# dzhang314/DZOptimization.jl

Measured on AMD Instinct MI355X. Metric: step!() calls/sec and achieved HBM GB/s, L-BFGS n=10^7 m=20 fp64, higher is better.
Workload: dtype f64

## Files before the change

### dzoptimization.jl_amd/__init__.py

```python
from __future__ import annotations

import ctypes as C
import os
import subprocess
import sys

import numpy as np

_HERE = os.path.dirname(os.path.abspath(__file__))
LIB_PATH = os.environ.get("DZO_LIB_PATH") or os.path.join(_HERE, "libdzo_hip.so")
INCLUDE_DIR = os.path.join(os.path.dirname(_HERE), "include")

F32, F64 = 0, 1
ROSENBROCK2D, ROSENBROCK_CHAIN, QUADRATIC, LSE, QUADRATIC_CHAIN = 0, 1, 2, 3, 4
PAIRWISE_LJ = 5
RADIAL_LENNARD_JONES = 0
RADIAL_MORSE_RHO6, RADIAL_MORSE_RHO14 = 2, 3
TWOLOOP_CHAIN, TWOLOOP_GRAM = 0, 1
LINE_SEARCH_BACKTRACKING, LINE_SEARCH_WOLFE = 0, 1
STEP_NULL, STEP_GRADIENT_DESCENT, STEP_BFGS = 0, 1, 2

_ERR = {1: "invalid argument", 2: "HIP runtime error", 3: "reference @assert", 4: "out of memory",
        5: "unsupported", 6: "bad call sequence", 7: "more candidates than the capacity"}

# ... 1915 lines not shown
    rho_history = property(lambda s: s._hist(lib().dzo_lbfgs_get_rho))
    alpha_history = property(lambda s: s._hist(lib().dzo_lbfgs_get_alpha))

    def set_two_loop_mode(self, mode):
        _check(lib().dzo_lbfgs_set_two_loop_mode(self.h, mode))

    def set_max_halvings(self, v):
        _check(lib().dzo_lbfgs_set_max_halvings(self.h, v))

    def set_safeguards(self, descent_check=False, steepest_descent_fallback=False):
        _check(lib().dzo_lbfgs_set_safeguards(self.h, int(descent_check), int(steepest_descent_fallback)))

    def set_line_search(self, kind, c1=0.0, c2=0.0, max_evals=0):
        _check(lib().dzo_lbfgs_set_line_search(self.h, int(kind), c1, c2, int(max_evals)))

    last_step_length = property(lambda s: s._s(2))
    history_resets = property(lambda s: s._i(8))
    descent_resets = property(lambda s: s._i(9))
    last_step_kind = property(lambda s: s._i(10))
    single_pass_steps = property(lambda s: s._i(11))
    single_pass_rejections = property(lambda s: s._i(12))
    single_pass_retries = property(lambda s: s._i(13))
    ring_layout = property(lambda s: s._i(14))
    tile_arrangement = property(lambda s: s._i(15))
    pass_recomputes_gradients = property(lambda s: bool(s._i(16)))
    pass_register_sets = property(lambda s: s._i(17))
    host_write_checks = property(lambda s: s._i(18))

    def compute_step_direction(self, sync=True):
        _check(lib().dzo_lbfgs_direction(self.h))
        return self.step_direction if sync else None

    def set_history(self, S, Y, rho=None, iteration_count=None):
        S, Y = _as_dev(S, self.dtype), _as_dev(Y, self.dtype)
        k = S.shape[0] if len(S.shape) == 2 else 0
        rp = None if rho is None else (C.c_double * k)(*[float(r) for r in rho])
        _check(lib().dzo_lbfgs_set_history(self.h, k, S.ptr, Y.ptr, rp, k if iteration_count is None else iteration_count))

    def begin_search(self):
        _check(lib().dzo_lbfgs_begin_search(self.h))

    def trial(self, t):
# ... 432 lines not shown
```

### dzoptimization.jl_amd/csrc/dzo_lbfgs.hip

```cpp
#include <cmath>
#include <cstdlib>
#include <limits>
#include <map>
#include <mutex>
#include <type_traits>
#include <utility>

#include "dzo_lbfgs_plan.h"
#include "dzo_optcore.h"
#include "dzo_rosen.h"

namespace dzo {

static_assert(kPlanWaves == kWaves && kPlanMaxHistory == kMaxHistory && kPlanMaxPartialBlocks == kMaxPartialBlocks,
              "dzo_lbfgs_plan.h restates these constants of dzo_common.h");

struct SlotMap {
    uint8_t slot[kMaxHistory];
};

}

struct dzo_lbfgs_s {
    dzo::OptCore core;
// ... 30 lines not shown
    int32_t wolfe_max_evals = 40;
    double last_step_length = 0;
    int64_t history_resets = 0, descent_resets = 0;
    int32_t last_step_kind = 0;
    bool reset_on_push = false;
    void *xt = nullptr, *gt = nullptr;
    bool single_pass = true;
    bool gram_ready = false;
    int gram_ready_grid = 0;
    bool scalars_ready = false;
    void *twin_slab = nullptr, *x_twin = nullptr, *g_twin = nullptr, *d_alloc = nullptr;
    void *x_user = nullptr, *g_user = nullptr;
    bool unsettled = false;
    std::recursive_mutex mu;
    int64_t single_pass_steps = 0, single_pass_rejections = 0, single_pass_retries = 0;
    bool fused_post = true;

    int device = 0;
    int32_t nslots = 0;
    int slot_of(int i) const { return ((newest - i) % nslots + nslots) % nslots; }
    int spare() const { return (newest + 1) % nslots; }
    int64_t pair_stride = 0;
    bool blocked = false;
    int64_t rowbytes = 0, ring_rows = 0;
    int64_t tile_stride = dzo::kTileBytes;
    size_t ring_bytes = 0;
    void *dx_lin = nullptr, *dg_lin = nullptr;
    bool lin_stale = false;
    void *export_slab = nullptr;
    bool points = false;
// ... 688 lines not shown
template <typename T> __device__ __forceinline__ T decor_grad(const PointDecor<T> &d, T g, T x) {
    const T g2 = dfma(d.two_lambda, x, g);
    g = d.l2_on ? g2 : g;
    const bool pushed_back = (x <= d.bg_lo && g >= (T)0) || (x >= d.bg_hi && g <= (T)0);
    return pushed_back ? (T)0 : g;
}
template <typename T> __device__ __forceinline__ T decor_clamp(const PointDecor<T> &d, T v) {
    return v < d.cons_lo ? d.cons_lo : (v > d.cons_hi ? d.cons_hi : v);
}

template <typename T> struct FusedParams {
    int64_t n;
    int k;
    int k_next;
    T t;
    T t_half;
    const T *x, *g;
    T *x_out, *g_out;
    T *d;
    const double *alpha, *coef, *scale;
    T *ring;
    uint32_t rowbytes;
    uint32_t soff[kFusedMaxK + 1];
    uint32_t new_off;
    uint32_t ystride;
    double *gram_partials;
    double *obj_partials;
    int32_t *changed;
    int nt_tiles;
    int stage_rows;
    int store_d;
    int prio;
    int leftover_even;
    int debug_skip;
    PointDecor<T> dec;
    T obj_lambda;
};

template <typename T> static inline bool fused_params_ok(const FusedParams<T> &fp, bool pair) {
    const bool common = fp.ring && fp.alpha && fp.coef && fp.scale && fp.gram_partials && fp.obj_partials && fp.changed && fp.rowbytes != 0 && fp.n > 0;
    return common && (!pair || (fp.x && fp.g && fp.x_out && fp.g_out && fp.d)) && (pair || fp.d);
}

// ... 82 lines not shown
#pragma unroll
        for (int i = K - 1; i >= 0; --i) {
            const T c = c_s[i];
#pragma unroll
            for (int j = 0; j < N; ++j) q[j] = dfma(c, sv[i][j], q[j]);
        }
        T xn[N];
#pragma unroll
        for (int j = 0; j < N; ++j) {
            xn[j] = dfma(p.t, q[j], xo[j]);
            diff |= owner && !is_equal(xn[j], xo[j]);
        }
        {
            T xh[N];
#pragma unroll
            for (int j = 0; j < N; ++j) xh[j] = dfma(p.t_half, q[j], xo[j]);
            const T xhnext = lane_next<T>(xh[0]);
#pragma unroll
            for (int j = 0; j < N; ++j) {
                const T xq = j + 1 < N ? xh[(j + 1) % N] : xhnext;
                if (owner && e0 + j + 1 < p.n) fobj_h += rosen_term<T>(xh[j], xq);
            }
        }
        const T xprev = lane_prev<T>(xn[N - 1]);
        const T xnext = lane_next<T>(xn[0]);
        T gn[N], sn[N], yn[N];
#pragma unroll
        for (int j = 0; j < N; ++j) {
            const T xp = j > 0 ? xn[(j + N - 1) % N] : xprev;
            const T xq = j + 1 < N ? xn[(j + 1) % N] : xnext;
            gn[j] = rosen_grad_elem<T>(e0 + j, p.n, xp, xn[j], xq);
// ... 130 lines not shown
    __shared__ int64_t stage_row_s[kWaves][40];
    extern __shared__ __attribute__((aligned(16))) char stage_lds[];
    const int lane = threadIdx.x & 63;
    const int wave = threadIdx.x >> 6;
    const int stage_rows = p.stage_rows;
    constexpr bool kWriteG = !(DZO_PP_REGRAD != 0 && !FIRST);
    constexpr int kStageTiles = kWriteG ? 2 : 1;
    char *stage = stage_lds + (size_t)wave * stage_rows * (kStageTiles * kTileBytes);
    int staged = 0;
    const int k = p.k, kn = p.k_next;
    if (threadIdx.x < K) {
        a_s[threadIdx.x] = threadIdx.x < k ? (T)(-p.alpha[threadIdx.x]) : (T)0;
        c_s[threadIdx.x] = threadIdx.x < k ? (T)(-p.coef[threadIdx.x]) : (T)0;
    }
    constexpr bool kRegrad = DZO_PP_REGRAD != 0 && !FIRST;
    __syncthreads();
    const bool scaled = k > 0;
    const T scale = scaled ? (T)p.scale[0] : (T)1;
    const int64_t nvec = (p.n + N - 1) / N;
    const int64_t rows = (nvec + kOwn - 1) / kOwn;
    const int64_t row_end = rows;
    const int64_t stride = (int64_t)gridDim.x * kWaves;
    const int pstride = (int)gridDim.x;
    const int pcol = (int)blockIdx.x;
    TreeSum<kGramValues * (K + 1)> dots;
    dots.init();
    double fobj = 0, fobj_h = 0;
    double fsq = 0, fsq_h = 0;
    bool diff = false;
    auto byte_offset = [&](int64_t row) -> uint32_t {
// ... 97 lines not shown
            }
            if (scaled) {
#pragma unroll
                for (int j = 0; j < N; ++j) q[j] = scale * q[j];
            }
#pragma unroll
            for (int i = K - 1; i >= 0; --i) {
                const T c = c_s[i];
#pragma unroll
                for (int j = 0; j < N; ++j) q[j] = dfma(c, xv[i][j] - xv[i + 1][j], q[j]);
            }
        }
        T xn[N];
#pragma unroll
        for (int j = 0; j < N; ++j) {
            xn[j] = dfma(p.t, q[j], xv[0][j]);
            diff |= owner && !is_equal(xn[j], xv[0][j]);
            if constexpr (DEC) { const T cl = decor_clamp<T>(p.dec, xn[j]); xn[j] = e0 + j < p.n ? cl : xn[j]; }
        }
        {
            T xh[N];
#pragma unroll
            for (int j = 0; j < N; ++j) {
                xh[j] = dfma(p.t_half, q[j], xv[0][j]);
                if constexpr (DEC) {
                    const T cl = decor_clamp<T>(p.dec, xh[j]); xh[j] = e0 + j < p.n ? cl : xh[j];
                    if (owner) fsq_h = __builtin_fma((double)xh[j], (double)xh[j], fsq_h);
                }
            }
            const T xhnext = lane_next0<T>(xh[0]);
#pragma unroll
            for (int j = 0; j < N; ++j) {
                const T xq = j + 1 < N ? xh[(j + 1) % N] : xhnext;
                if (owner && Obj::has_term(e0 + j, p.n)) fobj_h += Obj::term(rc[j], xh[j], xq);
            }
        }
        const T xprev = lane_prev0<T>(xn[N - 1]);
        const T xnext = lane_next0<T>(xn[0]);
        T gn[N], sn[N], yn[N];
// ... 142 lines not shown
        const double *wflat = &wacc[0][0][0];
        constexpr int ws = kGramValues * (kFusedMaxK + 1);
        const double r = (wflat[v] + wflat[ws + v]) + (wflat[2 * ws + v] + wflat[3 * ws + v]);
        p.gram_partials[(int64_t)v * pstride + pcol] = r;
    }
    block_raise_flag(diff, p.changed, &lds_flag);
    const double fo = block_sum(fobj, lds);
    const double fh = block_sum(fobj_h, lds);
    if (threadIdx.x == 0) { p.obj_partials[pcol] = fo; p.obj_partials[pstride + pcol] = fh; }
    if constexpr (DEC) {
        const double so = block_sum(fsq, lds);
        const double sh = block_sum(fsq_h, lds);
        if (threadIdx.x == 0) { p.obj_partials[2 * pstride + pcol] = so; p.obj_partials[3 * pstride + pcol] = sh; }
    }
    if ((p.debug_skip & 1024) && blockIdx.x < 1024) { if (lane == 0) g_dev_wave_times[(blockIdx.x * kWaves + wave) * 2 + 1] = wall_clock64(); }
}

constexpr int kLseMaxK = 24;
template <typename T> struct LseParams {
    int64_t n;
    int k, k_next;
    T t;
    T *ring;
    uint32_t rowbytes;
    uint32_t soff[kLseMaxK + 1];
    uint32_t new_off, c_off;
    uint8_t slot[kLseMaxK + 1];
    uint8_t new_slot;
    double *pscal;
    double lambda;
// ... 1273 lines not shown
    DeviceScope scope(o->device);
    DZO_TRY(lbfgs_settle(o));
    DZO_HIP(hipStreamSynchronize(o->core.stream));
    return DZO_OK;
}


template <typename P> static int32_t pass_trial_launch(OptCore &c, void (*kern)(P), int grid, size_t dyn_lds, const P &p, int attempt) {
    if (!c.flag_armed) DZO_HIP(hipMemsetAsync(c.flag(), 0, sizeof(int32_t), c.stream));
    c.flag_armed = false;
    DZO_TIMED(attempt == 0 ? "lbfgs_single_pass" : "lbfgs_single_pass_retry", c.stream);
    hipLaunchKernelGGL(kern, dim3(grid), dim3(kBlock), dyn_lds, c.stream, p);
    return DZO_OK;
}

static int32_t gram_reduce_decide_launch(dzo_lbfgs_s *o, int k_next, const double *obj_partials, int grid, const double *l2_partials) {
    OptCore &c = o->core;
    {
        DZO_TIMED("lbfgs_gram_reduce", c.stream);
        const int nvals = kGramValues * k_next;
        DecideArgs da = decide_args(c, obj_partials, grid, 1.0);
        da.partials2 = obj_partials + grid;
        if (l2_partials) { da.l2_partials = l2_partials; da.l2_partials2 = l2_partials + grid; da.l2_lambda = o->ring_dec.l2; }
        hipLaunchKernelGGL(gram_reduce_decide_kernel, dim3(nvals + 1), dim3(kBlock), 0, c.stream, (const double *)o->gram_partials, grid, gram_vals(o),
                           nvals, da);
        c.flag_armed = true;
    }
    DZO_HIP(hipGetLastError());
    return DZO_OK;
}

static int32_t next_scalars_gated(dzo_lbfgs_s *o, int k_next) {
    const int sv_newest = o->newest, sv_k = o->k;
    o->newest = o->spare(); o->k = k_next;
    const int32_t rc = gram_finish_launch(o, 0, true, gram_vals(o), true, o->core.status());
    o->newest = sv_newest; o->k = sv_k;
    return rc;
}
// ... 16 lines not shown
    if (v.k > 0) { o->d_stale = true; o->dview_k = v.k; o->dview_newest = v.newest; }
}

template <typename T> static void fused_fill_params(dzo_lbfgs_s *o, FusedParams<T> &fp, int k, int view_newest) {
    OptCore &c = o->core;
    memset(&fp, 0, sizeof(fp));
    fp.n = c.n; fp.k = k; fp.k_next = k < o->m ? k + 1 : o->m;
    fp.d = (T *)o->d;
    fp.ring = (T *)o->S; fp.rowbytes = (uint32_t)o->rowbytes;
    fp.new_off = ring_tile_off(o, o->spare()); fp.ystride = (uint32_t)o->tile_stride;
    fp.alpha = o->alpha; fp.coef = o->coef; fp.scale = o->scale;
    for (int j = 0; j <= kFusedMaxK; ++j) fp.soff[j] = ring_tile_off(o, ring_view_slot(o, view_newest, j < k ? j : k));
    fp.gram_partials = o->gram_partials;
    fp.obj_partials = c.problem->scratch;
    fp.changed = c.flag();
    fp.dec = point_decor<T>(o->ring_dec);
    fp.obj_lambda = (T)o->ring_obj_lambda;
}

template <typename T> static int32_t points_end_stuck(dzo_lbfgs_s *o, RingView view) {
    o->core.is_stuck = true;
    direction_pending(o, view);
    if (o->k > 0) {
        DZO_TRY(lbfgs_ensure_g(o, o->slot_of(0))); DZO_TRY(lbfgs_ensure_g(o, o->slot_of(1)));
        ring_gather_diff<T>(o, o->y_slot_v(o->slot_of(0)), o->y_slot_v(o->slot_of(1)), o->dg_lin);
    }
    ring_gather<T>(o, o->s_slot_v(o->newest), o->dx_lin);
    DZO_HIP(hipGetLastError());
    o->lin_stale = false;
    return DZO_OK;
// ... 30 lines not shown
    fp.obj_partials = c.problem->scratch;
    fp.changed = c.flag();
    fp.debug_skip = tune_int("DZO_TUNE_SP_DEBUG", 0);
    const int pass_k = pair_pass_k(o->m);
    void (*kern)(FusedParams<T>) = pass_k == 8 ? lbfgs_single_pass_kernel<T, 8>
                                   : pass_k == 16 ? lbfgs_single_pass_kernel<T, 16>
                                   : lbfgs_single_pass_kernel<T, 20>;
    if constexpr (std::is_same<T, double>::value) {
        if ((fp.debug_skip & 256) && o->m > 16) kern = lbfgs_single_pass_kernel<double, 20, true>;
    }
    const int grid = pass_grid(rows, (int64_t)ctx().cus * resident_blocks((const void *)kern), o->gram_grid, kPairPassGridCap);
    DZO_REQUIRE(fused_params_ok<T>(fp, true), DZO_ERR_STATE, "single-pass step: a null operand (ring %p, x %p, g %p, twins %p %p, d %p)",
                (void *)fp.ring, (const void *)fp.x, (const void *)fp.g, (void *)fp.x_out, (void *)fp.g_out, (void *)fp.d);
    double t = 1.0;
    for (int attempt = 0;; ++attempt) {
    fp.t = (T)t; fp.t_half = (T)round_to_dtype(c.dtype, t * 0.5);
    DZO_TRY(pass_trial_launch(c, kern, grid, 0, fp, attempt));
    DZO_TRY(gram_reduce_decide_launch(o, fp.k_next, fp.obj_partials, grid, nullptr));
    DZO_TRY(next_scalars_gated(o, fp.k_next));
    DZO_TRY(core_wait_decision(c));
    const int32_t status = c.host_status();
    if (attempt == 0) { c.last_trials = 0; o->single_pass_steps += 1; }
    if (status == 2) {
        c.is_stuck = true;
        if (o->lin_stale && o->k > 0) { ring_gather<T>(o, o->y_slot_v(o->newest), o->dg_lin); o->lin_stale = false; }
        DZO_HIP(hipMemcpyAsync(c.dx, c.x, (size_t)c.n * sizeof(T), hipMemcpyDeviceToDevice, c.stream));
        DZO_HIP(hipGetLastError());
        return DZO_OK;
    }
    c.last_trials += 1;
    if (status == 1) {
// ... 31 lines not shown
        DZO_PP(24, false, 2, true, 0) DZO_PP(16, false, 2, true, 0) DZO_PP(20, false, 2, true, 0) DZO_PP(12, false, 2, true, 0)
        DZO_PP(18, false, 1, false, 0) DZO_PP(20, false, 1, false, 0) DZO_PP(16, false, 1, false, 0) DZO_PP(14, false, 1, false, 0) DZO_PP(12, false, 1, false, 0) DZO_PP(10, false, 1, false, 0) DZO_PP(8, false, 1, false, 0) DZO_PP(6, false, 1, false, 0)
        DZO_PP(22, false, 2, false, 0) DZO_PP(24, false, 2, false, 0) DZO_PP(16, false, 2, false, 0) DZO_PP(20, false, 2, false, 0) DZO_PP(12, false, 2, false, 0) DZO_PP(8, false, 2, false, 0)
    } else {
        DZO_PP(8, true, 2, true, 0) DZO_PP(8, true, 2, false, 0) DZO_PP(8, true, 2, false, 1)
        DZO_PP(8, false, 1, false, 1) DZO_PP(12, false, 1, false, 1)
        DZO_PP(16, false, 2, false, 1) DZO_PP(20, false, 2, false, 1) DZO_PP(12, false, 2, false, 1)
        DZO_PP(8, false, 1, true, 0) DZO_PP(12, false, 1, true, 0)
        DZO_PP(16, false, 2, true, 0) DZO_PP(20, false, 2, true, 0) DZO_PP(12, false, 2, true, 0)
        DZO_PP(10, false, 1, false, 0) DZO_PP(12, false, 1, false, 0) DZO_PP(8, false, 1, false, 0) DZO_PP(6, false, 1, false, 0)
        DZO_PP(16, false, 2, false, 0) DZO_PP(20, false, 2, false, 0) DZO_PP(12, false, 2, false, 0) DZO_PP(8, false, 2, false, 0)
    }
#undef DZO_PP
    return nullptr;
}
template <typename T> static void (*point_pass_kernel_for(dzo_lbfgs_s *o, bool first))(FusedParams<T>) {
    return point_pass_kernel_of<T>(point_pass_variant(o->m, o->core.dtype, point_one_set(o->m, o->core.dtype, o->point_sets),
                                                      o->ring_dec.any(), o->ring_obj, first));
}

template <typename T> static int32_t lbfgs_materialize_d_t(dzo_lbfgs_s *o) {
    OptCore &c = o->core;
    hipStream_t s = c.stream;
    FusedParams<T> fp;
    fused_fill_params<T>(o, fp, o->dview_k, o->dview_newest);
    fp.k_next = 1; fp.t = (T)1; fp.t_half = (T)0.5;
    fp.store_d = 1;
    fp.debug_skip = 1 | 64;
    fp.stage_rows = 1;
    void (*kern)(FusedParams<T>) = point_pass_kernel_for<T>(o, false);
    DZO_REQUIRE(kern, DZO_ERR_STATE, "direction on demand: no point-pass kernel for history_length %d", o->m);
    const int grid = points_grid<T>(o, kern);
    DZO_REQUIRE(fused_params_ok<T>(fp, false), DZO_ERR_STATE, "direction on demand: a null operand (ring %p, d %p)", (void *)fp.ring, (void *)fp.d);
    {
        DZO_TIMED("lbfgs_direction_on_demand", s);
        hipLaunchKernelGGL(kern, dim3(grid), dim3(kBlock), 0, s, fp);
    }
    DZO_HIP(hipMemsetAsync(c.flag(), 0, sizeof(int32_t), s));
    c.flag_armed = true;
    DZO_HIP(hipGetLastError());
    o->d_stale = false;
// ... 35 lines not shown
        o->stage_kern = (const void *)kern; o->stage_bytes = stage_bytes;
    }
    if (o->stage_small && fp.stage_rows > point_stage_small_rows(pl.stage_tiles)) {
        fp.stage_rows = point_stage_small_rows(pl.stage_tiles);
        stage_bytes = point_stage_bytes(fp.stage_rows, pl.stage_tiles);
    }
    const int grid = points_grid<T>(o, kern, stage_bytes);
    const int pgrid = grid;
    DZO_REQUIRE(fused_params_ok<T>(fp, false), DZO_ERR_STATE, "point pass: a null operand (ring %p, d %p, scalars %p %p %p)",
                (void *)fp.ring, (void *)fp.d, (const void *)fp.alpha, (const void *)fp.coef, (const void *)fp.scale);
    o->d_stale = false;
    const RingView view{k, o->newest};
    const double *l2_partials = o->ring_dec.l2 != 0.0 ? fp.obj_partials + 2 * pgrid : nullptr;
    c.last_trials = 0;
    o->single_pass_steps += 1;
    int64_t halvings = 0;
    double t = 1.0;
    for (int attempt = 0;; ++attempt) {
        fp.t = (T)t; fp.t_half = (T)round_to_dtype(c.dtype, t * 0.5);
        DZO_TRY(pass_trial_launch(c, kern, grid, stage_bytes, fp, attempt));
        DZO_TRY(gram_reduce_decide_launch(o, fp.k_next, fp.obj_partials, pgrid, l2_partials));
        DZO_TRY(next_scalars_gated(o, fp.k_next));
        DZO_TRY(core_wait_decision(c));
        const int32_t status = c.host_status();
        if (status == 2) return points_end_stuck<T>(o, view);
        c.last_trials += 1;
        if (status == 1) {
            return points_accept(o, view, round_to_dtype(c.dtype, c.host[0]), (k == 0) || DZO_PP_REGRAD == 0);
        }
        if (attempt == 0) o->single_pass_rejections += 1;
        auto halve = [&]() -> bool {
            t = round_to_dtype(c.dtype, t * 0.5);
            return !(c.max_halvings > 0 && ++halvings >= c.max_halvings);
        };
        bool go_on = halve();
        const double f_half = round_to_dtype(c.dtype, c.host[1]);
        if (go_on && !(f_half < c.f)) {
            c.last_trials += 1;
            go_on = halve();
        }
        if (!go_on) return points_end_stuck<T>(o, view);
        o->single_pass_retries += 1;
    }
}

template <typename T> static void lse_fill_params(dzo_lbfgs_s *o, LseParams<T> &lp, int k, int view_newest) {
    OptCore &c = o->core;
    memset(&lp, 0, sizeof(lp));
    lp.n = c.n; lp.k = k; lp.k_next = k < o->m ? k + 1 : o->m;
// ... 292 lines not shown
int32_t dzo_lbfgs_destroy(dzo_lbfgs_t o) {
    if (!o) return DZO_OK;
    DeviceScope scope(o->device);
    if (o->core.stream && o->x_user) (void)lbfgs_settle(o);
    unsettled_retire(o);
    if (o->core.stream) (void)hipStreamSynchronize(o->core.stream);
    if (o->S) (void)hipFree(o->S);
    if (o->d_alloc) (void)hipFree(o->d_alloc);
    if (o->twin_slab) (void)hipFree(o->twin_slab);
    if (o->dx_lin) (void)hipFree(o->dx_lin);
    if (o->dg_lin) (void)hipFree(o->dg_lin);
    if (o->export_slab) (void)hipFree(o->export_slab);
    if (o->xt) (void)hipFree(o->xt);
    if (o->gt) (void)hipFree(o->gt);
    if (o->gram_ticket) (void)hipFree(o->gram_ticket);
    core_free(o->core);
    delete o;
    return DZO_OK;
}

int32_t dzo_lbfgs_create_callbacks(dzo_constraint_fn constraint, dzo_objective_fn objective, dzo_gradient_fn gradient,
                                   void *cb_ctx, int64_t n, int32_t history_length, int32_t dtype, void *x_dev,
                                   double initial_step_length, dzo_lbfgs_t *out) {
    DZO_TRY(require_init());
    DZO_REQUIRE(objective && gradient && x_dev && out, DZO_ERR_INVALID, "null argument");
    DZO_REQUIRE(dtype == DZO_F32 || dtype == DZO_F64, DZO_ERR_INVALID, "bad dtype %d", dtype);
    DZO_TRY(require_same_backend("LBFGSOptimizer", "src/DZOptimization.jl:410,420", x_dev, "initial_point", nullptr, ""));
    if (constraint) DZO_REQUIRE(constraint(cb_ctx, x_dev) != 0, DZO_ERR_ASSERT,
                                "@assert constraint_function!(initial_point) (src/DZOptimization.jl:412-414)");
    const double f0 = objective(cb_ctx, x_dev);
// ... 148 lines not shown
    switch (what) {
    case 0: *value = o->core.is_stuck ? 1 : 0; break;
    case 1: *value = o->core.iteration_count; break;
    case 2: *value = o->core.n; break;
    case 3: *value = o->m; break;
    case 4: *value = o->k; break;
    case 5: *value = o->core.last_trials; break;
    case 6: *value = o->mode; break;
    case 7: *value = o->core.dtype; break;
    case 8: *value = o->history_resets; break;
    case 9: *value = o->descent_resets; break;
    case 10: *value = o->last_step_kind; break;
    case 11: *value = o->single_pass_steps; break;
    case 12: *value = o->single_pass_rejections; break;
    case 13: *value = o->single_pass_retries; break;
    case 14: *value = o->points ? 2 : (o->blocked ? 1 : 0); break;
    case 15: *value = o->blocked ? (o->tile_stride == kTileBytes ? 1 : 2) : 0; break;
    case 16: *value = (o->points && DZO_PP_REGRAD != 0) ? 1 : 0; break;
    case 18: *value = o->host_write_checks; break;
    case 17: { int sets = 0; if (o->points) { sets = point_one_set(o->m, o->core.dtype, o->point_sets) ? 1 : 2; } *value = sets; break; }
    default: set_error("dzo_lbfgs_get_i: unknown field %d", what); return DZO_ERR_INVALID;
    }
    return DZO_OK;
}

int32_t dzo_lbfgs_get_s(dzo_lbfgs_t o, int32_t what, double *value) {
    DZO_REQUIRE(o && value, DZO_ERR_INVALID, "null argument");
    DZO_REQUIRE(what >= 0 && what <= 2, DZO_ERR_INVALID, "unknown field %d", what);
    *value = what == 0 ? o->core.f : what == 1 ? o->core.df : o->last_step_length;
    return DZO_OK;
// ... 11 lines not shown
    DZO_REQUIRE(o, DZO_ERR_INVALID, "null optimizer");
    DZO_REQUIRE(kind == DZO_LINE_SEARCH_BACKTRACKING || kind == DZO_LINE_SEARCH_WOLFE, DZO_ERR_INVALID,
                "unknown line search %d", kind);
    DZO_REQUIRE(!(c1 > 0 && c2 > 0) || c1 < c2, DZO_ERR_INVALID, "Wolfe constants need 0 < c1 < c2 < 1");
    DZO_REQUIRE(c2 < 1.0, DZO_ERR_INVALID, "Wolfe constants need 0 < c1 < c2 < 1");
    DeviceScope scope(o->device);
    o->line_search = kind;
    if (c1 > 0) o->wolfe_c1 = round_to_dtype(o->core.dtype, c1);
    if (c2 > 0) o->wolfe_c2 = round_to_dtype(o->core.dtype, c2);
    if (max_evals > 0) o->wolfe_max_evals = max_evals;
    return DZO_OK;
}

int32_t dzo_lbfgs_set_s(dzo_lbfgs_t o, int32_t what, double value) {
    DZO_REQUIRE(o, DZO_ERR_INVALID, "null optimizer");
    DZO_REQUIRE(what >= 0 && what <= 2, DZO_ERR_INVALID, "unknown field %d", what);
    (what == 0 ? o->core.f : what == 1 ? o->core.df : o->last_step_length) = round_to_dtype(o->core.dtype, value);
    return DZO_OK;
}

int32_t dzo_lbfgs_set_stuck(dzo_lbfgs_t o, int32_t is_stuck) {
    DZO_REQUIRE(o, DZO_ERR_INVALID, "null optimizer");
    o->core.is_stuck = is_stuck != 0;
    return DZO_OK;
}

static int32_t lbfgs_field_ptr(dzo_lbfgs_t o, int32_t what, int32_t idx, bool hand_out, void **ptr_dev) {
    DZO_TRY(lbfgs_settle(o, hand_out));
    if (what == 1 || what == 3) DZO_TRY(lbfgs_refresh_lin(o));
    if (what == 4) DZO_TRY(lbfgs_materialize_d(o));
    if ((what == 5 || what == 6) && o->blocked) {
// ... 221 lines not shown
```

### dzoptimization.jl_amd/csrc/dzo_lbfgs_plan.h

```cpp
#pragma once

#include <cstddef>
#include <cstdint>

#include "../../include/dzo.h"

namespace dzo {

constexpr int kPlanWaves = 4, kPlanMaxHistory = 64, kPlanMaxPartialBlocks = 2048;

constexpr int kGramValues = 5;
constexpr int kRowOwn = 62;
constexpr int kRowLead = (64 - kRowOwn) / 2;
constexpr int kTileBytes = 64 * 16;
constexpr int kPairMaxK = 20;
static inline int point_max_k(int32_t dtype) { return dtype == DZO_F64 ? 24 : 20; }
constexpr int kFusedMaxK = 24;
constexpr int kStreamU = 4;

static inline int64_t plan_dtype_size(int32_t dtype) { return dtype == DZO_F64 ? 8 : 4; }

struct RingDecor {
    double l2 = 0; bool bg_on = false; double bg_lo = 0, bg_hi = 0; bool cons_on = false; double cons_lo = 0, cons_hi = 0;
    bool any() const { return l2 != 0.0 || bg_on || cons_on; }
// ... 203 lines not shown
static inline int point_stage_small_rows(int stage_tiles) { return 14 / stage_tiles; }
static inline PointLaunch point_pass_launch(int64_t n, int32_t dtype, int m, int k, int point_sets, bool regrad,
                                            int stage_rows_knob, int prio_knob, int64_t plain_mb) {
    PointLaunch p;
    p.nt_tiles = 2 * n * plan_dtype_size(dtype) > (plain_mb << 20) ? 1 : 0;
    p.one_set = point_one_set(m, dtype, point_sets) && k > 0;
    p.prio = p.one_set ? (prio_knob != 0 ? 1 : 0) : 0;
    p.stage_tiles = (k == 0 || !regrad) ? 2 : 1;
    p.stage_max = (p.one_set ? 72 : 144) / (4 * p.stage_tiles);
    p.stage_rows = stage_rows_knob < 1 ? 1 : stage_rows_knob;
    if (p.stage_rows > p.stage_max) p.stage_rows = p.stage_max;
    p.stage_bytes = point_stage_bytes(p.stage_rows, p.stage_tiles);
    return p;
}

}
```

### dzoptimization.jl_amd/csrc/dzo_optcore.h

```cpp
#pragma once
#include "dzo_common.h"
#include "dzo_problems.h"

namespace dzo {

struct OptCore {
    int64_t n = 0;
    int32_t dtype = DZO_F64;
    hipStream_t stream = nullptr;

    dzo_constraint_fn constraint = nullptr;
    dzo_objective_fn objective = nullptr;
    dzo_gradient_fn gradient = nullptr;
    void *cb_ctx = nullptr;
    dzo_problem_s *problem = nullptr;
    bool box_on = false; double box_lo = 0, box_hi = 0;

    bool is_stuck = false;
    int64_t iteration_count = 0;
    void *x = nullptr;
    void *dx = nullptr;
    double f = 0;
    double df = 0;
    void *g = nullptr;
// ... 5 lines not shown
    double *host_dev = nullptr;
    bool flag_armed = false;
    double ticket = 0;
    int64_t max_halvings = 4096;
    int64_t last_trials = 0;
    bool search_open = false;
    bool defer_delta = false;
    int32_t (*speculative_tail)(void *self, const int32_t *gate) = nullptr;
    void *speculative_self = nullptr;
    hipEvent_t decided = nullptr;

    double *partials() const { return ws; }
    double *result() const { return ws + 2 * kMaxPartialBlocks; }
    int32_t *flag() const { return reinterpret_cast<int32_t *>(ws + 2 * kMaxPartialBlocks + 4); }
    int32_t *status() const { return reinterpret_cast<int32_t *>(ws + 2 * kMaxPartialBlocks + 3); }
    int32_t host_status() const { return reinterpret_cast<const int32_t *>(host + 3)[0]; }
    bool has_objective() const { return objective != nullptr || problem != nullptr; }
    bool has_gradient() const { return gradient != nullptr || problem != nullptr; }
};

int32_t core_alloc(OptCore &c);
void core_free(OptCore &c);

inline double round_to_dtype(int32_t dtype, double v) { return dtype == DZO_F32 ? (double)(float)v : v; }

int32_t core_begin_search(OptCore &c);
int32_t core_trial(OptCore &c, double t, const void *dir, bool fuse_objective, int32_t *changed,
                   double *f_new, bool *f_valid);
int32_t core_accept(OptCore &c, double f_new);
int32_t core_reject(OptCore &c);
// ... 6 lines not shown

struct DecideArgs {
    double *result;
    const double *partials;
    const double *partials2;
    int64_t count;
    double scale;
    int32_t *changed;
    double f_cur;
    int to_f32;
    int32_t *status;
    double *host_out;
    double ticket;
    const double *l2_partials = nullptr, *l2_partials2 = nullptr;
    double l2_lambda = 0;
};
DecideArgs decide_args(OptCore &c, const double *partials, int64_t count, double scale);

__device__ __forceinline__ void decide_body(const DecideArgs &a, double *lds) {
    double f_new;
    double f_second = 0;
    const int32_t ch_early = threadIdx.x == 0 ? *a.changed : 0;
    if (a.partials && a.partials2) {
        __shared__ double lds2[2 * kWaves];
        double v[2] = {0, 0}, out[2];
        for (int64_t i = threadIdx.x; i < a.count; i += kBlock) { v[0] += a.partials[i]; v[1] += a.partials2[i]; }
        block_sum_multi<2>(v, lds2, out);
        f_new = a.scale * out[0];
        f_second = a.scale * out[1];
        if (a.l2_partials) {
            double w[2] = {0, 0}, ss[2];
            for (int64_t i = threadIdx.x; i < a.count; i += kBlock) { w[0] += a.l2_partials[i]; w[1] += a.l2_partials2[i]; }
            block_sum_multi<2>(w, lds2, ss);
            if (a.to_f32) {
                f_new = (double)((float)f_new + (float)a.l2_lambda * (float)ss[0]);
                f_second = (double)((float)f_second + (float)a.l2_lambda * (float)ss[1]);
            } else {
// ... 8 lines not shown
            for (int64_t i = threadIdx.x; i < a.count; i += kBlock) v += a.partials[i];
            f_new = a.scale * block_sum(v, lds);
            if (threadIdx.x == 0) a.result[0] = f_new;
        } else {
            f_new = a.result[0];
        }
        if (a.partials2) {
            double v = 0;
            for (int64_t i = threadIdx.x; i < a.count; i += kBlock) v += a.partials2[i];
            f_second = a.scale * block_sum(v, lds);
        }
    }
    if (threadIdx.x == 0) {
        const double f_raw = f_new;
        if (a.to_f32) f_new = (double)(float)f_new;
        const int32_t ch = ch_early;
        int32_t st = 0;
        if (ch == 0) st = 2;
        else if (f_new < a.f_cur) st = 1;
        *a.status = st;
        *a.changed = 0;
        const unsigned long long sw = (unsigned long long)(uint32_t)st, cw = (unsigned long long)(uint32_t)ch;
        unsigned long long *ho = reinterpret_cast<unsigned long long *>(a.host_out);
        auto put = [&](int i, unsigned long long w) { __hip_atomic_store(ho + i, w, __ATOMIC_RELAXED, __HIP_MEMORY_SCOPE_SYSTEM); };
        put(0, seal_bits(f_raw));
        put(1, seal_bits(f_second));
        put(2, 0ull); put(5, 0ull);
        put(3, sw);
        put(4, cw);
        put(6, seal_bits(f_raw) ^ seal_bits(f_second) ^ sw ^ cw ^ seal_bits(a.ticket));
        put(7, seal_bits(a.ticket));
    }
}

}
```

Measured before the change: 2736.

## Add sampled point probe to predict full-step rejection and swap trial order

Adds a small sampling kernel that estimates the objective change at the full step over a strided subset of rows before the fused single-pass trial. If the probe predicts rejection, the pass evaluates the half step as the primary candidate and the full step as the secondary one. The decide logic is extended to handle swapped passes, including a false-alarm status that triggers a retry. A credit scheme arms the probe only for a while after a first-trial rejection. The aim is to avoid wasted full passes over the large history ring when the unit step keeps being rejected, at the cost of an extra small kernel launch and more complex control flow.

```diff
diff --git a/dzoptimization.jl_amd/__init__.py b/dzoptimization.jl_amd/__init__.py
--- a/dzoptimization.jl_amd/__init__.py
+++ b/dzoptimization.jl_amd/__init__.py
@@ -1953,6 +1953,9 @@
     def set_line_search(self, kind, c1=0.0, c2=0.0, max_evals=0):
         _check(lib().dzo_lbfgs_set_line_search(self.h, int(kind), c1, c2, int(max_evals)))
 
+    def set_point_probe(self, mode):
+        _check(lib().dzo_lbfgs_set_s(self.h, 3, float(mode)))
+
     last_step_length = property(lambda s: s._s(2))
     history_resets = property(lambda s: s._i(8))
     descent_resets = property(lambda s: s._i(9))
@@ -1965,6 +1968,10 @@
     pass_recomputes_gradients = property(lambda s: bool(s._i(16)))
     pass_register_sets = property(lambda s: s._i(17))
     host_write_checks = property(lambda s: s._i(18))
+    probe_runs = property(lambda s: s._i(19))
+    probe_hits = property(lambda s: s._i(20))
+    point_probe = property(lambda s: s._i(22))
+    probe_false_alarms = property(lambda s: s._i(21))
 
     def compute_step_direction(self, sync=True):
         _check(lib().dzo_lbfgs_direction(self.h))
diff --git a/dzoptimization.jl_amd/csrc/dzo_lbfgs.hip b/dzoptimization.jl_amd/csrc/dzo_lbfgs.hip
--- a/dzoptimization.jl_amd/csrc/dzo_lbfgs.hip
+++ b/dzoptimization.jl_amd/csrc/dzo_lbfgs.hip
@@ -68,6 +68,10 @@
     bool unsettled = false;
     std::recursive_mutex mu;
     int64_t single_pass_steps = 0, single_pass_rejections = 0, single_pass_retries = 0;
+    int probe_mode = dzo::kProbeRule;
+    int probe_credit = 0;
+    double *probe_ws = nullptr;
+    int64_t probe_runs = 0, probe_hits = 0, probe_false_alarms = 0;
     bool fused_post = true;
 
     int device = 0;
@@ -786,7 +790,7 @@
     int k;
     int k_next;
     T t;
-    T t_half;
+    T t_other;
     const T *x, *g;
     T *x_out, *g_out;
     T *d;
@@ -799,6 +803,10 @@
     double *gram_partials;
     double *obj_partials;
     int32_t *changed;
+    int probe_use;
+    int probe_blocks;
+    double *probe_partials;
+    int32_t *pass_mode;
     int nt_tiles;
     int stage_rows;
     int store_d;
@@ -911,7 +919,7 @@
         {
             T xh[N];
 #pragma unroll
-            for (int j = 0; j < N; ++j) xh[j] = dfma(p.t_half, q[j], xo[j]);
+            for (int j = 0; j < N; ++j) xh[j] = dfma(p.t_other, q[j], xo[j]);
             const T xhnext = lane_next<T>(xh[0]);
 #pragma unroll
             for (int j = 0; j < N; ++j) {
@@ -1072,6 +1080,19 @@
         c_s[threadIdx.x] = threadIdx.x < k ? (T)(-p.coef[threadIdx.x]) : (T)0;
     }
     constexpr bool kRegrad = DZO_PP_REGRAD != 0 && !FIRST;
+    T t_p = p.t, t_o = p.t_other;
+    if constexpr (!FIRST) {
+        int swapped = p.probe_use == kProbeUseSwap ? 1 : 0;
+        if (p.probe_use == kProbeUseRule) {
+            double ps = 0, pa = 0;
+            for (int i = lane; i < p.probe_blocks; i += 64) { ps += p.probe_partials[i]; pa += p.probe_partials[p.probe_blocks + i]; }
+            ps = wave_sum_all(ps); pa = wave_sum_all(pa);
+            swapped = probe_predicts_reject(ps, pa) ? 1 : 0;
+        }
+        swapped = __builtin_amdgcn_readfirstlane(swapped);
+        if (swapped) { t_p = p.t_other; t_o = p.t; }
+        if (swapped && blockIdx.x == 0 && threadIdx.x == 0) *p.pass_mode = 1;
+    }
     __syncthreads();
     const bool scaled = k > 0;
     const T scale = scaled ? (T)p.scale[0] : (T)1;
@@ -1199,7 +1220,7 @@
         T xn[N];
 #pragma unroll
         for (int j = 0; j < N; ++j) {
-            xn[j] = dfma(p.t, q[j], xv[0][j]);
+            xn[j] = dfma(t_p, q[j], xv[0][j]);
             diff |= owner && !is_equal(xn[j], xv[0][j]);
             if constexpr (DEC) { const T cl = decor_clamp<T>(p.dec, xn[j]); xn[j] = e0 + j < p.n ? cl : xn[j]; }
         }
@@ -1207,7 +1228,7 @@
             T xh[N];
 #pragma unroll
             for (int j = 0; j < N; ++j) {
-                xh[j] = dfma(p.t_half, q[j], xv[0][j]);
+                xh[j] = dfma(t_o, q[j], xv[0][j]);
                 if constexpr (DEC) {
                     const T cl = decor_clamp<T>(p.dec, xh[j]); xh[j] = e0 + j < p.n ? cl : xh[j];
                     if (owner) fsq_h = __builtin_fma((double)xh[j], (double)xh[j], fsq_h);
@@ -1380,6 +1401,96 @@
         if (threadIdx.x == 0) { p.obj_partials[2 * pstride + pcol] = so; p.obj_partials[3 * pstride + pcol] = sh; }
     }
     if ((p.debug_skip & 1024) && blockIdx.x < 1024) { if (lane == 0) g_dev_wave_times[(blockIdx.x * kWaves + wave) * 2 + 1] = wall_clock64(); }
+}
+
+template <typename T, int K, bool DEC, int OBJ>
+__global__ __launch_bounds__(kBlock) void lbfgs_point_probe_kernel(FusedParams<T> p, int64_t row_stride) {
+    using Obj = ChainObj<T, OBJ>;
+    constexpr int N = Vec16<T>::N;
+    constexpr int kOwn = kRowOwn, kLead = kRowLead;
+    __shared__ T a_s[kFusedMaxK], c_s[kFusedMaxK];
+    __shared__ double rowsum_s[kWaves];
+    const int lane = threadIdx.x & 63;
+    const int wave = threadIdx.x >> 6;
+    const int k = p.k;
+    if (threadIdx.x < K) {
+        a_s[threadIdx.x] = threadIdx.x < k ? (T)(-p.alpha[threadIdx.x]) : (T)0;
+        c_s[threadIdx.x] = threadIdx.x < k ? (T)(-p.coef[threadIdx.x]) : (T)0;
+    }
+    __syncthreads();
+    const T scale = (T)p.scale[0];
+    const int64_t nvec = (p.n + N - 1) / N;
+    const int64_t rows = (nvec + kOwn - 1) / kOwn;
+    const int64_t row = ((int64_t)blockIdx.x * kWaves + wave) * row_stride;
+    double dsum = 0;
+    if (row < rows) {
+        const int64_t v = row * kOwn - kLead + lane;
+        const bool owner = v >= 0 && v < nvec && lane >= kLead && lane < kLead + kOwn;
+        const int64_t e0 = v * N;
+        const char *rb = reinterpret_cast<const char *>(p.ring) + (uint64_t)row * p.rowbytes + (uint32_t)lane * 16u;
+        T xv[K + 1][N], gv[K + 1][N];
+#pragma unroll
+        for (int j = 0; j <= K; ++j) load16_nt(reinterpret_cast<const T *>(rb + p.soff[j]), xv[j]);
+        typename Obj::Coef rc[N];
+#pragma unroll
+        for (int e = 0; e < N; ++e) rc[e] = Obj::coef(e0 + e, p.n, p.obj_lambda);
+#pragma unroll
+        for (int j = 0; j <= K; ++j) {
+            const T xp = lane_prev0<T>(xv[j][N - 1]);
+            const T xq = lane_next0<T>(xv[j][0]);
+#pragma unroll
+            for (int e = 0; e < N; ++e) {
+                const T xl = e > 0 ? xv[j][(e + N - 1) % N] : xp;
+                const T xr = e + 1 < N ? xv[j][(e + 1) % N] : xq;
+                gv[j][e] = Obj::grad(rc[e], xl, xv[j][e], xr);
+                if constexpr (DEC) gv[j][e] = decor_grad<T>(p.dec, gv[j][e], xv[j][e]);
+            }
+        }
+        T q[N];
+#pragma unroll
+        for (int j = 0; j < N; ++j) q[j] = gv[0][j];
+#pragma unroll
+        for (int i = 0; i < K; ++i) {
+            const T a = a_s[i];
+#pragma unroll
+            for (int j = 0; j < N; ++j) q[j] = dfma(a, gv[i][j] - gv[i + 1][j], q[j]);
+        }
+#pragma unroll
+        for (int j = 0; j < N; ++j) q[j] = scale * q[j];
+#pragma unroll
+        for (int i = K - 1; i >= 0; --i) {
+            const T c = c_s[i];
+#pragma unroll
+            for (int j = 0; j < N; ++j) q[j] = dfma(c, xv[i][j] - xv[i + 1][j], q[j]);
+        }
+        T xn[N];
+#pragma unroll
+        for (int j = 0; j < N; ++j) {
+            xn[j] = dfma(p.t, q[j], xv[0][j]);
+            if constexpr (DEC) { const T cl = decor_clamp<T>(p.dec, xn[j]); xn[j] = e0 + j < p.n ? cl : xn[j]; }
+        }
+        const T xnnext = lane_next0<T>(xn[0]);
+        const T x0next = lane_next0<T>(xv[0][0]);
+        const double l2 = DEC && p.dec.l2_on ? 0.5 * (double)p.dec.two_lambda : 0.0;
+#pragma unroll
+        for (int j = 0; j < N; ++j) {
+            const T xq = j + 1 < N ? xn[(j + 1) % N] : xnnext;
+            const T x0q = j + 1 < N ? xv[0][(j + 1) % N] : x0next;
+            if (owner && Obj::has_term(e0 + j, p.n)) dsum += Obj::term(rc[j], xn[j], xq) - Obj::term(rc[j], xv[0][j], x0q);
+            if constexpr (DEC) {
+                if (owner && e0 + j < p.n) dsum += l2 * ((double)xn[j] * (double)xn[j] - (double)xv[0][j] * (double)xv[0][j]);
+            }
+        }
+    }
+    const double rowsum = wave_sum_all(dsum);
+    if (lane == 0) rowsum_s[wave] = rowsum;
+    __syncthreads();
+    if (threadIdx.x == 0) {
+        double s = 0, a = 0;
+        for (int w = 0; w < kWaves; ++w) { s += rowsum_s[w]; a += fabs(rowsum_s[w]); }
+        p.probe_partials[blockIdx.x] = s;
+        p.probe_partials[p.probe_blocks + blockIdx.x] = a;
+    }
 }
 
 constexpr int kLseMaxK = 24;
@@ -2683,7 +2794,8 @@
     return DZO_OK;
 }
 
-static int32_t gram_reduce_decide_launch(dzo_lbfgs_s *o, int k_next, const double *obj_partials, int grid, const double *l2_partials) {
+static int32_t gram_reduce_decide_launch(dzo_lbfgs_s *o, int k_next, const double *obj_partials, int grid, const double *l2_partials,
+                                         bool point_pass = false) {
     OptCore &c = o->core;
     {
         DZO_TIMED("lbfgs_gram_reduce", c.stream);
@@ -2691,6 +2803,7 @@
         DecideArgs da = decide_args(c, obj_partials, grid, 1.0);
         da.partials2 = obj_partials + grid;
         if (l2_partials) { da.l2_partials = l2_partials; da.l2_partials2 = l2_partials + grid; da.l2_lambda = o->ring_dec.l2; }
+        if (point_pass) da.pass_mode = c.pass_mode();
         hipLaunchKernelGGL(gram_reduce_decide_kernel, dim3(nvals + 1), dim3(kBlock), 0, c.stream, (const double *)o->gram_partials, grid, gram_vals(o),
                            nvals, da);
         c.flag_armed = true;
@@ -2737,6 +2850,7 @@
     fp.gram_partials = o->gram_partials;
     fp.obj_partials = c.problem->scratch;
     fp.changed = c.flag();
+    fp.pass_mode = c.pass_mode();
     fp.dec = point_decor<T>(o->ring_dec);
     fp.obj_lambda = (T)o->ring_obj_lambda;
 }
@@ -2797,7 +2911,7 @@
                 (void *)fp.ring, (const void *)fp.x, (const void *)fp.g, (void *)fp.x_out, (void *)fp.g_out, (void *)fp.d);
     double t = 1.0;
     for (int attempt = 0;; ++attempt) {
-    fp.t = (T)t; fp.t_half = (T)round_to_dtype(c.dtype, t * 0.5);
+    fp.t = (T)t; fp.t_other = (T)round_to_dtype(c.dtype, t * 0.5);
     DZO_TRY(pass_trial_launch(c, kern, grid, 0, fp, attempt));
     DZO_TRY(gram_reduce_decide_launch(o, fp.k_next, fp.obj_partials, grid, nullptr));
     DZO_TRY(next_scalars_gated(o, fp.k_next));
@@ -2859,6 +2973,23 @@
 #undef DZO_PP
     return nullptr;
 }
+template <typename T> static void (*point_probe_kernel_of(PassVariant v))(FusedParams<T>, int64_t) {
+#define DZO_PB(K_, DEC_, OBJ_) \
+    if (v.K == K_ && v.DEC == DEC_ && v.OBJ == OBJ_) return lbfgs_point_probe_kernel<T, K_, DEC_, OBJ_>;
+    if (v.FIRST) return nullptr;
+    if constexpr (sizeof(T) == 8) {
+        DZO_PB(8, false, 1) DZO_PB(12, false, 1) DZO_PB(16, false, 1) DZO_PB(20, false, 1) DZO_PB(24, false, 1)
+        DZO_PB(8, true, 0) DZO_PB(12, true, 0) DZO_PB(16, true, 0) DZO_PB(20, true, 0) DZO_PB(24, true, 0)
+        DZO_PB(6, false, 0) DZO_PB(8, false, 0) DZO_PB(10, false, 0) DZO_PB(12, false, 0) DZO_PB(14, false, 0) DZO_PB(16, false, 0)
+        DZO_PB(18, false, 0) DZO_PB(20, false, 0) DZO_PB(22, false, 0) DZO_PB(24, false, 0)
+    } else {
+        DZO_PB(8, false, 1) DZO_PB(12, false, 1) DZO_PB(16, false, 1) DZO_PB(20, false, 1)
+        DZO_PB(8, true, 0) DZO_PB(12, true, 0) DZO_PB(16, true, 0) DZO_PB(20, true, 0)
+        DZO_PB(6, false, 0) DZO_PB(8, false, 0) DZO_PB(10, false, 0) DZO_PB(12, false, 0) DZO_PB(16, false, 0) DZO_PB(20, false, 0)
+    }
+#undef DZO_PB
+    return nullptr;
+}
 template <typename T> static void (*point_pass_kernel_for(dzo_lbfgs_s *o, bool first))(FusedParams<T>) {
     return point_pass_kernel_of<T>(point_pass_variant(o->m, o->core.dtype, point_one_set(o->m, o->core.dtype, o->point_sets),
                                                       o->ring_dec.any(), o->ring_obj, first));
@@ -2869,7 +3000,7 @@
     hipStream_t s = c.stream;
     FusedParams<T> fp;
     fused_fill_params<T>(o, fp, o->dview_k, o->dview_newest);
-    fp.k_next = 1; fp.t = (T)1; fp.t_half = (T)0.5;
+    fp.k_next = 1; fp.t = (T)1; fp.t_other = (T)0.5;
     fp.store_d = 1;
     fp.debug_skip = 1 | 64;
     fp.stage_rows = 1;
@@ -2935,25 +3066,70 @@
     const double *l2_partials = o->ring_dec.l2 != 0.0 ? fp.obj_partials + 2 * pgrid : nullptr;
     c.last_trials = 0;
     o->single_pass_steps += 1;
+    const int probe_mode_now = o->probe_mode;
+    void (*probe_kern)(FusedParams<T>, int64_t) = nullptr;
+    const ProbeLaunch prl = probe_launch((ring_nvec<T>(o) + kRowOwn - 1) / kRowOwn);
+    bool probe_now = probe_armed(ProbeState{probe_mode_now, o->probe_credit, c.max_halvings, k});
+    if (probe_now) {
+        probe_kern = point_probe_kernel_of<T>(point_pass_variant(o->m, c.dtype, point_one_set(o->m, c.dtype, o->point_sets), o->ring_dec.any(), o->ring_obj, false));
+        DZO_REQUIRE(probe_kern, DZO_ERR_STATE, "point pass: no probe kernel for history_length %d", o->m);
+        if (!o->probe_ws) DZO_HIP(hipMalloc((void **)&o->probe_ws, sizeof(double) * 2 * kProbeMaxBlocks));
+        fp.probe_partials = o->probe_ws; fp.probe_blocks = prl.blocks;
+    }
+    bool first_known = false;
     int64_t halvings = 0;
     double t = 1.0;
     for (int attempt = 0;; ++attempt) {
-        fp.t = (T)t; fp.t_half = (T)round_to_dtype(c.dtype, t * 0.5);
+        fp.t = (T)t; fp.t_other = (T)round_to_dtype(c.dtype, t * 0.5);
+        fp.probe_use = probe_use_of(probe_mode_now, probe_now);
+        if (probe_now) {
+            DZO_TIMED("lbfgs_point_probe", c.stream);
+            hipLaunchKernelGGL(probe_kern, dim3(prl.blocks), dim3(kBlock), 0, c.stream, fp, prl.row_stride);
+            o->probe_runs += 1;
+        }
         DZO_TRY(pass_trial_launch(c, kern, grid, stage_bytes, fp, attempt));
-        DZO_TRY(gram_reduce_decide_launch(o, fp.k_next, fp.obj_partials, pgrid, l2_partials));
+        DZO_TRY(gram_reduce_decide_launch(o, fp.k_next, fp.obj_partials, pgrid, l2_partials, true));
         DZO_TRY(next_scalars_gated(o, fp.k_next));
         DZO_TRY(core_wait_decision(c));
         const int32_t status = c.host_status();
+        const uint32_t flags = reinterpret_cast<const uint32_t *>(c.host + 4)[0];
+        const bool swapped = probe_now && (flags & 4u) != 0;
+        probe_now = false;
+        if (swapped && status == 3) {
+            o->probe_false_alarms += 1;
+            o->probe_credit = probe_credit_after(o->probe_credit, false, true);
+            first_known = true;
+            attempt = -1;
+            continue;
+        }
+        if (swapped) o->probe_hits += 1;
+        if (!first_known) {
+            first_known = true;
+            const bool first_rejected = swapped || status == 0;
+            o->probe_credit = probe_credit_after(o->probe_credit, first_rejected, false);
+        }
+        if (swapped) {
+            c.last_trials += 1;
+            o->single_pass_rejections += 1;
+            t = round_to_dtype(c.dtype, t * 0.5);
+            halvings += 1;
+        }
         if (status == 2) return points_end_stuck<T>(o, view);
         c.last_trials += 1;
         if (status == 1) {
             return points_accept(o, view, round_to_dtype(c.dtype, c.host[0]), (k == 0) || DZO_PP_REGRAD == 0);
         }
-        if (attempt == 0) o->single_pass_rejections += 1;
+        if (attempt == 0 && !swapped) o->single_pass_rejections += 1;
         auto halve = [&]() -> bool {
             t = round_to_dtype(c.dtype, t * 0.5);
             return !(c.max_halvings > 0 && ++halvings >= c.max_halvings);
         };
+        if (swapped) {
+            if (c.max_halvings > 0 && halvings >= c.max_halvings) return points_end_stuck<T>(o, view);
+            if (!halve()) return points_end_stuck<T>(o, view);
+            o->single_pass_retries += 1;
+            continue;
+        }
         bool go_on = halve();
         const double f_half = round_to_dtype(c.dtype, c.host[1]);
         if (go_on && !(f_half < c.f)) {
@@ -3276,6 +3452,7 @@
     if (o->xt) (void)hipFree(o->xt);
     if (o->gt) (void)hipFree(o->gt);
     if (o->gram_ticket) (void)hipFree(o->gram_ticket);
+    if (o->probe_ws) (void)hipFree(o->probe_ws);
     core_free(o->core);
     delete o;
     return DZO_OK;
@@ -3454,6 +3631,10 @@
     case 11: *value = o->single_pass_steps; break;
     case 12: *value = o->single_pass_rejections; break;
     case 13: *value = o->single_pass_retries; break;
+    case 19: *value = o->probe_runs; break;
+    case 20: *value = o->probe_hits; break;
+    case 21: *value = o->probe_false_alarms; break;
+    case 22: *value = o->probe_mode; break;
     case 14: *value = o->points ? 2 : (o->blocked ? 1 : 0); break;
     case 15: *value = o->blocked ? (o->tile_stride == kTileBytes ? 1 : 2) : 0; break;
     case 16: *value = (o->points && DZO_PP_REGRAD != 0) ? 1 : 0; break;
@@ -3495,7 +3676,12 @@
 
 int32_t dzo_lbfgs_set_s(dzo_lbfgs_t o, int32_t what, double value) {
     DZO_REQUIRE(o, DZO_ERR_INVALID, "null optimizer");
-    DZO_REQUIRE(what >= 0 && what <= 2, DZO_ERR_INVALID, "unknown field %d", what);
+    DZO_REQUIRE(what >= 0 && what <= 3, DZO_ERR_INVALID, "unknown field %d", what);
+    if (what == 3) {
+        DZO_REQUIRE(value == 0.0 || value == 1.0 || value == 2.0 || value == 3.0, DZO_ERR_INVALID, "point-probe mode %g is not 0, 1, 2 or 3", value);
+        o->probe_mode = (int)value;
+        return DZO_OK;
+    }
     (what == 0 ? o->core.f : what == 1 ? o->core.df : o->last_step_length) = round_to_dtype(o->core.dtype, value);
     return DZO_OK;
 }
diff --git a/dzoptimization.jl_amd/csrc/dzo_lbfgs_plan.h b/dzoptimization.jl_amd/csrc/dzo_lbfgs_plan.h
--- a/dzoptimization.jl_amd/csrc/dzo_lbfgs_plan.h
+++ b/dzoptimization.jl_amd/csrc/dzo_lbfgs_plan.h
@@ -241,4 +241,36 @@
     return p;
 }
 
-}
+constexpr double kProbeRejectRatio = 0.5 * (0.8197 + -0.7095);
+constexpr bool probe_predicts_reject(double sum, double abs_sum) { return sum > 0 && sum > kProbeRejectRatio * abs_sum; }
+
+enum ProbeMode { kProbeOff = 0, kProbeRule = 1, kProbeAlwaysSwap = 2, kProbeIgnore = 3 };
+constexpr int kProbeCredit = 32;
+struct ProbeState {
+    int mode = kProbeRule;
+    int credit = 0;
+    int64_t max_halvings = 4096;
+    int k = 0;
+};
+static inline bool probe_armed(const ProbeState &s) {
+    if (s.mode == kProbeOff || s.max_halvings == 1 || s.k < 1) return false;
+    return s.mode == kProbeAlwaysSwap || s.mode == kProbeIgnore || s.credit > 0;
+}
+static inline int probe_credit_after(int credit, bool first_rejected, bool false_alarm) {
+    return false_alarm ? 0 : first_rejected ? kProbeCredit : (credit > 0 ? credit - 1 : 0);
+}
+enum ProbeUse { kProbeUseNone = 0, kProbeUseRule = 1, kProbeUseSwap = 2 };
+static inline int probe_use_of(int mode, bool armed) {
+    return !armed ? kProbeUseNone : mode == kProbeAlwaysSwap ? kProbeUseSwap : mode == kProbeIgnore ? kProbeUseNone : kProbeUseRule;
+}
+constexpr int kProbeRowStride = 39, kProbeMaxBlocks = 512;
+struct ProbeLaunch { int blocks; int64_t row_stride; };
+static inline ProbeLaunch probe_launch(int64_t rows) {
+    int64_t blocks = rows / ((int64_t)kProbeRowStride * kPlanWaves);
+    if (blocks < 1) blocks = 1;
+    if (blocks > kProbeMaxBlocks) blocks = kProbeMaxBlocks;
+    int64_t stride = rows / (blocks * kPlanWaves);
+    return {(int)blocks, stride < 1 ? 1 : stride};
+}
+
+}
diff --git a/dzoptimization.jl_amd/csrc/dzo_optcore.h b/dzoptimization.jl_amd/csrc/dzo_optcore.h
--- a/dzoptimization.jl_amd/csrc/dzo_optcore.h
+++ b/dzoptimization.jl_amd/csrc/dzo_optcore.h
@@ -43,6 +43,7 @@
     double *result() const { return ws + 2 * kMaxPartialBlocks; }
     int32_t *flag() const { return reinterpret_cast<int32_t *>(ws + 2 * kMaxPartialBlocks + 4); }
     int32_t *status() const { return reinterpret_cast<int32_t *>(ws + 2 * kMaxPartialBlocks + 3); }
+    int32_t *pass_mode() const { return reinterpret_cast<int32_t *>(ws + 2 * kMaxPartialBlocks + 8); }
     int32_t host_status() const { return reinterpret_cast<const int32_t *>(host + 3)[0]; }
     bool has_objective() const { return objective != nullptr || problem != nullptr; }
     bool has_gradient() const { return gradient != nullptr || problem != nullptr; }
@@ -79,6 +80,7 @@
     double ticket;
     const double *l2_partials = nullptr, *l2_partials2 = nullptr;
     double l2_lambda = 0;
+    int32_t *pass_mode = nullptr;
 };
 DecideArgs decide_args(OptCore &c, const double *partials, int64_t count, double scale);
 
@@ -86,6 +88,7 @@
     double f_new;
     double f_second = 0;
     const int32_t ch_early = threadIdx.x == 0 ? *a.changed : 0;
+    const int32_t swapped = (threadIdx.x == 0 && a.pass_mode) ? *a.pass_mode : 0;
     if (a.partials && a.partials2) {
         __shared__ double lds2[2 * kWaves];
         double v[2] = {0, 0}, out[2];
@@ -124,12 +127,21 @@
     if (threadIdx.x == 0) {
         const double f_raw = f_new;
         if (a.to_f32) f_new = (double)(float)f_new;
-        const int32_t ch = ch_early;
+        int32_t ch = ch_early;
         int32_t st = 0;
+        if (swapped) {
+            const double f_other = a.to_f32 ? (double)(float)f_second : f_second;
+            if (ch == 0) st = 3;
+            else if (f_other < a.f_cur) st = 3;
+            else if (f_new < a.f_cur) st = 1;
+            ch = (ch != 0 ? 1 : 0) | 4;
+        } else {
         if (ch == 0) st = 2;
         else if (f_new < a.f_cur) st = 1;
+        }
         *a.status = st;
         *a.changed = 0;
+        if (a.pass_mode) *a.pass_mode = 0;
         const unsigned long long sw = (unsigned long long)(uint32_t)st, cw = (unsigned long long)(uint32_t)ch;
         unsigned long long *ho = reinterpret_cast<unsigned long long *>(a.host_out);
         auto put = [&](int i, unsigned long long w) { __hip_atomic_store(ho + i, w, __ATOMIC_RELAXED, __HIP_MEMORY_SCOPE_SYSTEM); };
```

Result: slower. 2637 (-3.6%).
